# lucidrains/transfusion-pytorch

Measured on AMD Instinct MI355X. Metric: train samples/sec, dim512 d8 seq1024 text+latent, higher is better.
Workload: dtype bf16; 1 GPU; BASELINE config 2: Transfusion dim=512 depth=8 heads=8 dim_head=64 num_text_tokens=256 dim_latent=384; per-GPU batch 64 x seq 1024 (32 x [24 text tokens + (4,384) latent] per sample); step = pack + fwd + bwd + clip(0.5) + Adam(3e-4) (one GPU: no gradient exchange); global_batch=64, seq_len=1024, parallelism=dp1

## Files before the change

### include/tfx.h

```cpp
#ifndef TFX_H
#define TFX_H
#include <stdint.h>
#ifdef __cplusplus
extern "C" {
#endif

#ifndef TFX_BF16_DEFINED
typedef uint16_t tfx_bf16;
#endif

enum { TFX_EPI_BF16 = 0, TFX_EPI_F32 = 1, TFX_EPI_SILU = 2, TFX_EPI_RESID = 3, TFX_EPI_GEGLU = 4, TFX_EPI_GEGLU_BWD = 5, TFX_EPI_QKV_NORM_ROPE = 6 };

typedef struct {
  const tfx_bf16* A; int32_t lda;
  const tfx_bf16* A2; int32_t lda2; int32_t K1;
  const tfx_bf16* B; int32_t ldb;
  int32_t M, N, K;
  int32_t epi;
  void* C; int32_t ldc;
  void* C2; int32_t ldc2;
  const float* bias;
  const tfx_bf16* R; int32_t ldr; int32_t resid_mapped;
  const int32_t* rowmap;
  const int32_t* a_rowmap;
// ... 6 lines not shown
  tfx_bf16* qk_cache; int32_t qk_ld_cache; const int32_t* qk_cache_pos;
  const void* prefetch; int64_t prefetch_bytes;
} tfx_gemm_nt_args;
int tfx_gemm_nt(const tfx_gemm_nt_args* a, void* stream);
int tfx_gemm_nt_plan(const tfx_gemm_nt_args* a, int32_t* kind, int32_t* grid);

int tfx_mfma_peak_probe(const void* ops, float* out, int32_t iters, int32_t blocks, void* stream);

typedef struct {
  const tfx_bf16* A; int32_t lda; int32_t a_cols;
  const tfx_bf16* B; int32_t ldb; int32_t b_cols;
  int32_t M, N, K;
  float* C; int32_t ldc;
  const int32_t* rowmap;
  int32_t k_valid;
  int32_t splits;
  int32_t accumulate;
  float alpha;
  const int32_t* a_rowmap;
  const int32_t* b_rowmap;
  float* colsum;
  int32_t k_group;
  const void* group_next;
} tfx_gemm_tn_args;
int tfx_gemm_tn(const tfx_gemm_tn_args* a, void* stream);
int tfx_gemm_tn_plan(const tfx_gemm_tn_args* a, int32_t* kind, int32_t* tiles, int32_t* splits, int32_t* grid);

typedef struct {
  const tfx_bf16 *q, *k, *v; int32_t ld_q, ld_k, ld_v;
  const tfx_bf16* gate; int32_t ld_gate;
  const int32_t* kv_end;
  const int32_t* q_start;
  tfx_bf16* out; int32_t ld_out;
  float* lse;
  int32_t b, h, n;
  float softcap;
  int32_t n_kv;
  const tfx_bf16* dout; int32_t ld_dout;
  tfx_bf16* do_eff; int32_t ld_do;
  float* delta;
  tfx_bf16* dgate; int32_t ld_dgate;
  tfx_bf16 *dq, *dk, *dv; int32_t ld_dq, ld_dk, ld_dv;
  int32_t order;
  const float* sc_plan;
  const int32_t* q_row0; const int32_t* q_cnt;
  const tfx_bf16* nr_qkv; int32_t nr_ld_qkv;
// ... 296 lines not shown
```

### transfusion_pytorch_amd/csrc/gemm.hip

```cpp
#include "tfx_common.h"
#include "tfx_kernels.h"
#include <type_traits>
#include <cmath>
#include <cstring>
#include <vector>
#include <algorithm>
#include <mutex>

namespace tfx {

constexpr int BM = 128, BN = 128, BK = 64;

template <int EPI> struct Epilogue;

TFX_DEV void store_bf16x4(bf16* dst, f32x4 v) {
  bf16x4 o; o[0] = f2bf(v[0]); o[1] = f2bf(v[1]); o[2] = f2bf(v[2]); o[3] = f2bf(v[3]);
  *(bf16x4*)dst = o;
}

TFX_DEV f32x4 add_bias(const GemmNT& p, int n, f32x4 v) {
  if (p.bias) { f32x4 b = *(const f32x4*)(p.bias + n); v += b; }
  return v;
}

// ... 1884 lines not shown
#pragma unroll
      for (int j = 0; j < 4; j++)
        if (out_col[j] >= 0) atomicAdd(crow + out_col[j], acc[i][j][r] * p.alpha);
    }
  }
}
template <bool SUM>
__global__ __launch_bounds__(256, 1) void gemm_tn_ow_kernel(GemmTN p, int ramp) {
  const int ntn = (p.N + 255) / 256, ntk = (p.K + 255) / 256;
  tn_ow_body<SUM>(p, tn_block_ramp(p, ntn * ntk, ramp));
}
constexpr int TN_GROUP_MAX = 6;
struct TnGroup { int count; int tile_end[TN_GROUP_MAX]; GemmTN p[TN_GROUP_MAX]; };
template <bool SUM>
__global__ __launch_bounds__(256, 1) void gemm_tn_ow_group_kernel(TnGroup g, int ramp) {
  TnBlock blk = tn_block_ramp(g.p[0], g.tile_end[g.count - 1], ramp);
  int pid = 0, first = 0;
#pragma unroll
  for (int i = 0; i < TN_GROUP_MAX - 1; i++)
    if (i + 1 < g.count && blk.tile >= g.tile_end[i]) { pid = i + 1; first = g.tile_end[i]; }
  blk.tile -= first;
  tn_ow_body<SUM>(g.p[__builtin_amdgcn_readfirstlane(pid)], blk);
}
#undef OWT_OUT
#undef OWT_IN
#undef OWT_CLOBBER

static int tn_auto_splits(int M, int tiles, int kind) {
  constexpr double fill2 = 0.9, fill0 = 0.5;
  const int slots = kind == 2 ? 256 : 512;
  const double want = (kind == 2 ? fill2 : fill0) * slots;
  int s = 1;
  while (tiles * s < want && tiles * (s + 1) <= slots && s < 64 && M / (s + 1) >= 256) s++;
  return s;
}

static bool use_glds() {
  static int v = -1;
  if (v < 0) { const char* e = getenv("TFX_GEMM_GLDS"); v = (e && e[0] == '0') ? 0 : 1; }
  return v == 1;
}

enum { NT_FALLBACK = 0, NT_GLDS = 1, NT_MID = 2, NT_PP = 3, NT_SKINNY = 4, NT_DECODE = 5, NT_OW = 6, NT_OWP = 7 };

static const float* gelu_table() {
  static const float* tab[16] = {nullptr};
// ... 220 lines not shown
  const GemmTN* q = &head;
  int n = 0, tiles = 0;
  bool ok = grp != 0 && tn_ow_mode() != 0;
  while (q && n < TN_GROUP_MAX) {
    ok = ok && q->M == head.M && tn_ow_operands_ok(*q);
    tiles += ((q->N + 255) / 256) * ((q->K + 255) / 256);
    gp.g.p[n] = *q; gp.g.p[n].group_next = nullptr; gp.g.tile_end[n] = tiles;
    n++;
    q = (const GemmTN*)q->group_next;
  }
  ok = ok && q == nullptr && n >= 2;
  gp.count = n; gp.tiles = tiles; gp.g.count = n;
  if (!ok) return gp;
  gp.splits = head.splits == 0 ? tn_auto_splits(head.M, tiles, 2) : head.splits;
  const int chunk = ((head.M + gp.splits - 1) / gp.splits + TN_BMK - 1) / TN_BMK * TN_BMK;
  const int last = head.M % chunk == 0 ? chunk : head.M % chunk;
  if (chunk < 192 || last < 192) return gp;
  gp.grid = (tiles * gp.splits + 7) / 8 * 8;
  if (head.splits == 0 && tiles * gp.splits < 0.8 * 256) return gp;
  for (int i = 0; i < n; i++) gp.g.p[i].splits = gp.splits;
  gp.ok = true;
  return gp;
}
static int tn_ramp(int M, int tiles, int splits) {
  constexpr int ramp_min = 8;
  int ramp = 0;
  if (splits >= ramp_min && M % TN_BMK == 0) {
    const int S = splits, U = M / TN_BMK;
    ramp = (int)(0.148 * tiles + 0.5);
    while (ramp > 0 && (U - ramp * S * (S - 1) / 2) / S < 8) ramp--;
  }
  return ramp;
}

int gemm_tn_plan(const GemmTN& p, int* kind, int* tiles, int* splits, int* grid) {
  if (p.M <= 0 || p.N <= 0 || p.K <= 0 || p.splits < 0) return -1;
  if (p.group_next) {
    const TnGroupPlan gp = tn_group_plan(p);
    if (gp.ok) { if (kind) *kind = 3; if (tiles) *tiles = gp.tiles; if (splits) *splits = gp.splits; if (grid) *grid = gp.grid; return 0; }
  }
  const TnPlan pl = tn_plan(p);
  if (kind) *kind = pl.kind; if (tiles) *tiles = pl.tiles; if (splits) *splits = pl.splits; if (grid) *grid = pl.grid;
  return 0;
}

int gemm_tn(const GemmTN& p, hipStream_t s) {
  if (p.M <= 0 || p.N <= 0 || p.K <= 0 || p.splits < 0) return -1;
  if ((p.lda | p.ldb | p.a_cols | p.b_cols) & 7) return -2;
  if (p.group_next) {
    const TnGroupPlan gp = tn_group_plan(p);
    if (gp.ok) {
      bool sum = false;
      for (int i = 0; i < gp.count; i++) sum = sum || gp.g.p[i].colsum != nullptr;
      const int ramp = tn_ramp(p.M, gp.tiles, gp.splits);
      static uint32_t attr_g0 = 0, attr_g1 = 0;
      if (sum) { ensure_smem_attr((const void*)gemm_tn_ow_group_kernel<true>, 131072, attr_g1); hipLaunchKernelGGL(gemm_tn_ow_group_kernel<true>, dim3(gp.grid), dim3(256), 131072, s, gp.g, ramp); }
      else { ensure_smem_attr((const void*)gemm_tn_ow_group_kernel<false>, 131072, attr_g0); hipLaunchKernelGGL(gemm_tn_ow_group_kernel<false>, dim3(gp.grid), dim3(256), 131072, s, gp.g, ramp); }
      return (int)hipGetLastError();
    }
    int guard = 0;
    for (const GemmTN* q = &p; q; q = (const GemmTN*)q->group_next) {
      if (++guard > 64) return -7;
      GemmTN one = *q; one.group_next = nullptr;
      const int rc = gemm_tn(one, s);
      if (rc) return rc;
    }
    return 0;
  }
  static uint32_t attr_set = 0;
  const int smem = 2 * 2 * TN_BMK * TN_LD * 2;
  ensure_smem_attr((const void*)gemm_tn_kernel, smem, attr_set);
// ... 32 lines not shown
```

### transfusion_pytorch_amd/csrc/runner.hip

```cpp
#include <atomic>
#include <hip/hip_runtime.h>
#include <cstdlib>
#include <cstdint>
#include "../../include/tfx.h"

namespace {

inline int run_one(const tfx_launch& l, void* s) {
  const void* a = l.args;
  const tfx_raw_args* r = static_cast<const tfx_raw_args*>(a);
  switch (l.op) {
    case TFX_OP_GEMM_NT:          return tfx_gemm_nt(static_cast<const tfx_gemm_nt_args*>(a), s);
    case TFX_OP_GEMM_TN:          return tfx_gemm_tn(static_cast<const tfx_gemm_tn_args*>(a), s);
    case TFX_OP_ATTN_FWD:         return tfx_attn_fwd(static_cast<const tfx_attn_args*>(a), s);
    case TFX_OP_ATTN_BWD:         return tfx_attn_bwd(static_cast<const tfx_attn_args*>(a), s);
    case TFX_OP_ADALN_PRE_FWD:    return tfx_adaln_pre_fwd(static_cast<const tfx_adaln_pre_args*>(a), s);
    case TFX_OP_ADALN_PRE_BWD:    return tfx_adaln_pre_bwd(static_cast<const tfx_adaln_pre_args*>(a), s);
    case TFX_OP_ADALN_POST_FWD:   return tfx_adaln_post_fwd(static_cast<const tfx_adaln_post_args*>(a), s);
    case TFX_OP_ADALN_POST_BWD:   return tfx_adaln_post_bwd(static_cast<const tfx_adaln_post_args*>(a), s);
    case TFX_OP_QK_NORM_ROPE_FWD: return tfx_qk_norm_rope_fwd(static_cast<const tfx_qk_norm_rope_args*>(a), s);
    case TFX_OP_QK_NORM_ROPE_BWD: return tfx_qk_norm_rope_bwd(static_cast<const tfx_qk_norm_rope_args*>(a), s);
    case TFX_OP_ATTNRES_FWD:      return tfx_attnres_fwd(static_cast<const tfx_attnres_args*>(a), s);
    case TFX_OP_ATTNRES_BWD:      return tfx_attnres_bwd(static_cast<const tfx_attnres_args*>(a), s);
    case TFX_OP_RMSNORM_FWD:      return tfx_rmsnorm_fwd(static_cast<const tfx_rmsnorm_args*>(a), s);
// ... 192 lines not shown
extern "C" int tfx_list_fingerprint(const tfx_launch* list, int32_t n, int64_t* out) {
  if (!out || n < 0 || (n > 0 && !list)) return -1;
  uint64_t h = 1469598103934665603ull ^ (g_single_stream.load(std::memory_order_relaxed) ? 0x9e3779b97f4a7c15ull : 0ull);
  for (int32_t i = 0; i < n; ++i) {
    const tfx_launch& l = list[i];
    h = mix(h, &l.op, 4); h = mix(h, &l.stream, 4);
    if (l.op >= TFX_OP_FORK && l.op <= TFX_OP_JOIN_WAIT) continue;
    if (!l.args) return -2;
    const size_t nb = struct_bytes(l.op);
    if (nb == 0) return -100;
    h = mix(h, l.args, nb);
    const tfx_raw_args* r = static_cast<const tfx_raw_args*>(l.args);
    switch (l.op) {
      case TFX_OP_ADALN_POST_PRE_FWD: h = mix(h, r->p0, sizeof(tfx_adaln_post_args)); h = mix(h, r->p1, sizeof(tfx_adaln_pre_args)); break;
      case TFX_OP_LAYER_END_FWD:
        h = mix(h, r->p0, sizeof(tfx_adaln_post_args)); h = mix(h, r->p1, sizeof(tfx_attnres_args));
        if (r->p2) h = mix(h, r->p2, sizeof(tfx_adaln_pre_args));
        break;
      case TFX_OP_ATTNRES_PULL_BWD: h = mix(h, r->p0, sizeof(tfx_attnres_pull_args)); if (r->p1) h = mix(h, r->p1, sizeof(tfx_adaln_post_args)); break;
      case TFX_OP_ADALN_PRE_POST_BWD: h = mix(h, r->p0, sizeof(tfx_adaln_pre_args)); h = mix(h, r->p1, sizeof(tfx_adaln_post_args)); break;
      case TFX_OP_GEMM_TN: {
        const tfx_gemm_tn_args* g = static_cast<const tfx_gemm_tn_args*>(l.args);
        for (int k = 0; k < 8 && g->group_next; ++k) { g = static_cast<const tfx_gemm_tn_args*>(g->group_next); h = mix(h, g, sizeof(tfx_gemm_tn_args)); }
        break;
      }
      default: break;
    }
  }
  *out = (int64_t)h;
  return 0;
}

extern "C" int tfx_set_single_stream(int32_t on) {
  const int prev = g_single_stream.exchange(on != 0) ? 1 : 0;
  return prev;
}
```

### transfusion_pytorch_amd/csrc/tokenwise.hip

```cpp
#include "tfx_kernels.h"
#include <map>
#include <mutex>
#include <utility>
#include <cstdlib>

namespace tfx {

constexpr int WAVES = 4;
constexpr int MAXB = 1024;

template <int NC> struct Row {
  float v[NC][8];
};

template <int NC> TFX_DEV void load_row(Row<NC>& r, const bf16* p, int d, int lane) {
#pragma unroll
  for (int i = 0; i < NC; i++) {
    int c = lane + 64 * i;
    if (c * 8 < d) {
      bf16x8 x = *(const bf16x8*)(p + c * 8);
#pragma unroll
      for (int e = 0; e < 8; e++) r.v[i][e] = bf2f(x[e]);
    } else {
#pragma unroll
// ... 2324 lines not shown
int tfx_attn_fwd(const tfx_attn_args* a, void* s) { return attn_fwd(*a, ST(s)); }
int tfx_attn_bwd(const tfx_attn_args* a, void* s) { return attn_bwd(*a, ST(s)); }
int tfx_mfma_peak_probe(const void* ops, float* out, int32_t iters, int32_t blocks, void* s) {
  if (!ops || !out || iters <= 0 || blocks <= 0) return -1;
  hipLaunchKernelGGL(mfma_peak_k, dim3(blocks), dim3(256), 0, ST(s), (const bf16x8*)ops, out, iters); RET();
}
int tfx_laser_v_fwd(const tfx_laser_v_args* a, void* s) {
  if (!a || a->T < 0 || a->H <= 0 || !(a->c > 0.f)) return -1;
  if (a->T == 0) return 0;
  if (!a->v || !a->vl || ((a->ld_v | a->ld_vl) & 7) || a->ld_v < a->H * 64 || a->ld_vl < a->H * 64 || (((uintptr_t)a->v | (uintptr_t)a->vl) & 15)) return -2;
  const long long nch = (long long)a->T * a->H * 8;
  if (nch >= (1ll << 31)) return -4;
  hipLaunchKernelGGL(laser_v_fwd_k, dim3((unsigned)((nch + 255) / 256)), dim3(256), 0, ST(s), *a, (unsigned)nch); RET();
}
int tfx_laser_v_bwd(const tfx_laser_v_args* a, void* s) {
  if (!a || a->T < 0 || a->H <= 0 || !(a->c > 0.f)) return -1;
  if (a->T == 0) return 0;
  if (!a->v || !a->dvl || !a->dv || ((a->ld_v | a->ld_dvl | a->ld_dv) & 7) || a->ld_v < a->H * 64 || a->ld_dvl < a->H * 64 || a->ld_dv < a->H * 64 ||
      (((uintptr_t)a->v | (uintptr_t)a->dvl | (uintptr_t)a->dv) & 15)) return -2;
  const long long nch = (long long)a->T * a->H * 8;
  if (nch >= (1ll << 31)) return -4;
  hipLaunchKernelGGL(laser_v_bwd_k, dim3((unsigned)((nch + 255) / 256)), dim3(256), 0, ST(s), *a, (unsigned)nch); RET();
}
const char* tfx_version(void) { return "tfx-hip gfx950 r5-laser-muon-selfflow-adamgroups-oderk"; }

}
```

### transfusion_pytorch_amd/engine.py

```python
from __future__ import annotations

import ctypes
import os
import weakref

import torch

from . import capi
from .params import ModelDims, ParamStore, pad_to

BF16 = torch.bfloat16
E = capi.ENUMS


def _p(t, *idx):
    for i in idx:
        t = t[i]
    return t.data_ptr()


def skip_sources(md: ModelDims):
    stack, src = [], {}
    for i in range(md.depth):
        layer = i + 1
# ... 114 lines not shown
                    arr[k].stream = int(a)
                    arr[k].args = ctypes.addressof(_DUMMY)
                    continue
                arr[k].stream = 1 if isinstance(item, Side) else 0
                if isinstance(fn, str):
                    arr[k].op = capi.ENUMS['TFX_OP_' + fn[4:].upper()]
                    arr[k].args = ctypes.addressof(a)
                else:
                    name = fn.__name__
                    r = raw_args(name, a)
                    keep.append(r)
                    if isinstance(a, list):
                        live.append((name, a, r))
                    arr[k].op = capi.ENUMS['TFX_OP_' + name[4:].upper()]
                    arr[k].args = ctypes.addressof(r)
            self._image = (len(self), arr, keep, live)
        for name, a, r in self._image[3]:
            fresh = raw_args(name, a)
            ctypes.memmove(ctypes.addressof(r), ctypes.addressof(fresh), ctypes.sizeof(_RAW))
        return self._image[1]


class Plan:
    def __init__(self, ps: ParamStore, b: int, n: int, I: int, R: dict, training: bool = True, cache=None, dp_groups: int = 0, tile_attn: bool = False, units=None, ctl_rows: int = 2):
        md = ps.md
        self.units = units
        assert not units or (cache is not None and tile_attn), 'compacted plans are decode plans on the tiled attention kernel (the row ranges are its arguments)'
        self.cache = cache
        self.tile_attn = tile_attn
        assert cache is None or not training
        self.dp_groups = dp_groups
        self.bwd_cuts = []
        self.ps, self.md, self.b, self.n, self.I, self.R = ps, md, b, n, I, dict(R)
        self.T = T = b * n
        dev = ps.device
        d, hd, D, dip, ldq, nt3 = md.dim, md.hdk, md.depth, md.dip, md.ldq, md.nt3
        self.nbytes = 0
        def z(*s, dtype=BF16):
            t = torch.zeros(*s, device=dev, dtype=dtype); self.nbytes += t.numel() * t.element_size(); return t
        def e(*s, dtype=BF16):
            t = torch.empty(*s, device=dev, dtype=dtype); self.nbytes += t.numel() * t.element_size(); return t
        I1 = max(I, 1)
        self.idx = z(7, max(T, 1, 4 * units[0] if units else 1), dtype=torch.int32)
        self.text_ids, self.cache_pos, self.kv_end, self.rot_pos, self.tok_inst, self.q_start, self.labels = (self.idx[r, :T] if r != 1 else self.idx[r] for r in range(7))
        if units:
            U = units[0]
            self.unit_row0, self.unit_cnt, self.unit_blk0, self.unit_txt = (self.idx[6, k * U:(k + 1) * U] for k in range(4))
        self.inst_time = z(I1, dtype=torch.float32)
        self.row_tok = {t: z(r, dtype=torch.int32) for t, r in R.items()}
        self.rowbuf = None
        if cache is not None and R and len(set(R.values())) == 1:
            r = next(iter(R.values()))
            self.row_stride = rs = (r + 3) // 4 * 4
            self.rowbuf = z(2 * len(R) * rs + ctl_rows * max(b, units[0] if units else 0), dtype=torch.int32)
            self.row_tok = {t: self.rowbuf[k * rs:k * rs + r] for k, t in enumerate(R)}
# ... 42 lines not shown
                self.vl = e(nl, T, hd)
            else:
                side = ps.__dict__.setdefault('_laser_side', weakref.WeakValueDictionary())
                key = (cache.data_ptr(), tuple(cache.shape), tuple(cache.stride()))
                self.vlc = side.get(key)
                if self.vlc is None:
                    self.vlc = e(D, cache.shape[1] * cache.shape[2], hd)
                    side[key] = self.vlc
        self.fwd, self.bwd = LaunchList(), LaunchList()
        self.noise_args = {}
        self.loaded_structure = None
        self._seg_args = []
        self.seg_start = z(max(T, 1), dtype=torch.int32); self.seg_len = z(max(T, 1), dtype=torch.int32)
        self.pull = training and D <= 32 and md.dim <= 1024
        if self.pull:
            self.arsave = [e(T, i + 2, 4, dtype=torch.float32) for i in range(D)]
            self.arerr = e(D, T, d)
        self._build_forward()
        if training:
            self.dH = e(D + 1, T, d)
            self.gx = {i: e(T, d) for i in range(D) if md.has_skip(i)}; self.du = e(T, d)
            env = os.environ.get('TFX_SIDE_STREAM')
            self.side = D <= 30 and (env == '1' or (env is None and md.dim <= 1024))
            nb = 2 if self.side else 1
            self.dy_f = [e(T, d) for _ in range(nb)]; self.dy_a = [e(T, d) for _ in range(nb)] if self.side else self.dy_f
            self.dskip = {j: e(T, d) for j in set(skip_sources(md).values())}
            self.dqkvg_p = [z(T, ldq) for _ in range(nb)]; self.dog = e(T, hd); self.do_eff = e(T, hd)
            self.dqk = e(T, 2 * hd) if os.environ.get('TFX_ATTN_QKNR', '1') == '0' else None
            self.delta = e(b, md.heads, n, dtype=torch.float32)
            self.dag_p = [e(T, 2 * dip) for _ in range(nb)]; self.dembed = e(T, d); self.gfin = e(T, d); self.dx0 = e(T, d)
            self.dtables = z(I1, nt3, dtype=torch.float32); self.dtab_bf = e(I1, nt3)
            self.dcond = e(I1, 4 * d); self.dpre = e(I1, 4 * d)
            self.onehot = e(T, md.vp)
            self._build_backward()

    def _nt(self, lst, algo_n=None, algo_k=None, **kw):
        a = capi.make_args('tfx_gemm_nt_args', **kw)
        a._algo_flops = 2.0 * kw['M'] * (algo_n or kw['N']) * (algo_k or kw['K'])
        lst.append(('tfx_gemm_nt', a))

    def _tn(self, lst, M, N, K, **kw):
        splits = 0
        kw.setdefault('k_valid', K)
        algo_n = kw.pop('algo_n', None)
        side = kw.pop('side', False)
        a = capi.make_args('tfx_gemm_tn_args', M=M, N=N, K=K, splits=splits, accumulate=1, alpha=1.0, **kw)
        a._algo_flops = 2.0 * M * (algo_n or N) * kw['k_valid']
        lst.append(Side(('tfx_gemm_tn', a)) if side else ('tfx_gemm_tn', a))

    def _tn_group(self, lst, M, problems, side=False):
        if len(problems) < 2 or os.environ.get('TFX_TN_GROUP', '1') == '0':
            for (N, K, kw) in problems:
                self._tn(lst, M, N, K, side=side, **kw)
            return
        structs, flops = [], 0.0
        for (N, K, kw) in problems:
            kw = dict(kw); kw.setdefault('k_valid', K)
            algo_n = kw.pop('algo_n', None)
            a = capi.make_args('tfx_gemm_tn_args', M=M, N=N, K=K, splits=0, accumulate=1, alpha=1.0, **kw)
            flops += 2.0 * M * (algo_n or N) * kw['k_valid']
            structs.append(a)
        for a, b in zip(structs, structs[1:]):
            a.group_next = ctypes.addressof(b)
        head = structs[0]
        head._chain = structs[1:]
        head._algo_flops = flops
        lst.append(Side(('tfx_gemm_tn', head)) if side else ('tfx_gemm_tn', head))

    def _k(self, lst, fn, struct, **kw):
        lst.append((fn, capi.make_args(struct, **kw)))

    def _raw(self, lst, fn, *args):
        lst.append((fn, args))

    def _hbm(self, lst, passes, extra_bytes=0):
        if lst.meta is None:
            lst.meta = {}
        lst.meta[len(lst) - 1] = ('hbm', passes * self.T * self.md.dim * 2 + extra_bytes)

    def _tab(self, i, w):
        off = ((i * 2 + w) * 3 * self.md.dim) * 4
        return self.tables.data_ptr() + off, (self.dtables.data_ptr() + off if hasattr(self, 'dtables') else 0)

    def _build_forward(self):
        ps, md, T, I = self.ps, self.md, self.T, self.I
        d, hd, D, dip, ldq, nt3, H = md.dim, md.hdk, md.depth, md.dip, md.ldq, md.nt3, md.heads
        S = ps.shadows
        L = self.fwd
        pp = ps.ptr
        if self.cache is not None:
# ... 220 lines not shown
        assert mode in ('latent', 'model')
        self.clean_mode = mode
        for t, a in self._clean_launch.items():
            lt = self.lat[t]
            a[1] = lt['q'].data_ptr() if mode == 'model' else lt['x'].data_ptr()
            a[2] = None if mode == 'model' else self.noise_args[t].eps

    def _attn_kw(self, i, bwd=False):
        md, hd, ldq = self.md, self.md.hdk, self.md.ldq
        li, lkv = self._li(i), self._lkv(i)
        kw = dict(q=self.qkr[lkv], k=_p(self.qkr, lkv) + 2 * hd, v=_p(self.qkvg, lkv) + 2 * 2 * hd, ld_q=2 * hd, ld_k=2 * hd, ld_v=ldq,
                  gate=_p(self.qkvg, lkv) + 2 * 3 * hd, ld_gate=ldq, kv_end=self.kv_end, q_start=self.q_start, out=self.og[li], ld_out=hd,
                  lse=self.lse[li], b=self.units[0] if self.units else self.b, h=md.heads, n=self.units[1] if self.units else self.n, softcap=50.0)
        if self.units:
            kw.update(q_row0=self.unit_row0, q_cnt=self.unit_cnt)
        if self.sc_plan is not None:
            kw['sc_plan'] = self.sc_plan[i]
        if self.cache is not None:
            ck = self.cache[i]
            kw.update(k=ck.data_ptr(), v=ck.data_ptr() + 2 * hd, ld_k=2 * hd, ld_v=2 * hd, n_kv=int(ck.shape[1]))
        if md.laser:
            kw.update(v=self.vl[li] if self.cache is None else self.vlc[i], ld_v=hd, laser=1)
        if bwd:
            dqkvg = self.dqkvg_p[i % len(self.dqkvg_p)]
            kw.update(dout=self.dog, ld_dout=hd, do_eff=self.do_eff, ld_do=hd, delta=self.delta,
                      dgate=dqkvg.data_ptr() + 2 * 3 * hd, ld_dgate=ldq, dq=self.dqk if self.dqk is not None else 0,
                      dk=self.dqk.data_ptr() + 2 * hd if self.dqk is not None else 0,
                      dv=dqkvg.data_ptr() + 2 * 2 * hd, ld_dq=2 * hd, ld_dk=2 * hd, ld_dv=ldq)
        return kw

    def set_rope_tables(self, cos_tab, sin_tab):
        if self.cos_tab is not None and (self.cos_tab.data_ptr() != cos_tab.data_ptr() or self.sin_tab.data_ptr() != sin_tab.data_ptr()):
            self.fwd.invalidate_graphs()
        self.cos_tab, self.sin_tab = cos_tab, sin_tab
        for a in getattr(self, '_rope_args', []):
            a.cos_tab, a.sin_tab = cos_tab.data_ptr(), sin_tab.data_ptr()
        for a in getattr(self, '_rope_nt_args', []):
            a.qk_cos, a.qk_sin = cos_tab.data_ptr(), sin_tab.data_ptr()
        for a in getattr(self, '_rope_attn_args', []):
            a.nr_cos, a.nr_sin = cos_tab.data_ptr(), sin_tab.data_ptr()

    def set_segments(self, seg_start, seg_len):
        n_seg = int(seg_start.numel())
        self.seg_start[:n_seg].copy_(seg_start); self.seg_len[:n_seg].copy_(seg_len)
        for a in self._seg_args:
            a.n_seg = n_seg

# ... 107 lines not shown
                                 pq=pp(f'{pj}.pseudo_queries'), dgamma=gp(f'{pj}.norm_keys.gamma'), dpq=gp(f'{pj}.pseudo_queries'), L=j + 2).items():
                    setattr(recs[j], k, v.data_ptr() if hasattr(v, 'data_ptr') else v)
            raw = torch.frombuffer(bytearray(ctypes.string_at(ctypes.addressof(recs), ctypes.sizeof(recs))), dtype=torch.uint8)
            self._src_tab = raw.to(ps.device)
            self._src_size = ctypes.sizeof(SRC)
            self._raw(L, lib.tfx_attnres_prep, self._src_tab.data_ptr(), D, d)
        self._pull_args = {}
        def pull_launch(l, out_own, add, dh, post):
            j0 = max(l - 1, 0)
            ns = D - j0
            export = ns > 8 or d > 512
            if export and not hasattr(self, 'k1buf'):
                self.k1buf = torch.zeros(T, 32, device=ps.device, dtype=BF16); self.nbytes += self.k1buf.numel() * 2
            a = capi.make_args('tfx_attnres_pull_args', T=T, d=d, l=l, n_src=ns, h=self.hid[l], src=self._src_tab.data_ptr() + j0 * self._src_size,
                               out_own=out_own, out_err=self.arerr[l - 1] if out_own is not None else None, add=add, dh=dh,
                               seg_start=self.seg_start, seg_len=self.seg_len, n_seg=0, k1=self.k1buf if export else None, ld_k1=32)
            self._seg_args.append(a)
            self._pull_args[l] = a
            self._keep = getattr(self, '_keep', []) + [a, post]
            self._raw(L, lib.tfx_attnres_pull_bwd, ctypes.addressof(a), ctypes.addressof(post) if post is not None else None)
            self._hbm(L, ns + 6 if post is not None else ns + 4, 12 * ns * T)
            if export:
                self._tn(L, T, ns, d, A=self.k1buf, lda=32, a_cols=32, B=self.hid[l], ldb=d, b_cols=d, C=self.wtab[1, j0], ldc=d)
        for i in range(D - 1, -1, -1):
            p = f'transformer.layers.{i}'
            x_in = self.xres[i]
            x_a = self.xa[i] if md.has_skip(i) else x_in
            (ta, dta), (tf, dtf) = self._tab(i, 0), self._tab(i, 1)
            par = i % len(self.dag_p)
            dy_f, dy_a, dag, dqkvg = self.dy_f[par], self.dy_a[par], self.dag_p[par], self.dqkvg_p[par]
            if i + 2 <= D - 1:
                sync('tfx_join_wait', i + 2)
            G = self.dH[i + 1]
            a_postf = capi.make_args('tfx_adaln_post_args', T=T, d=d, y=self.yf[i], tok_inst=self.tok_inst, table=tf, ld_table=nt3,
                                     layerscale=pp(f'{p}.2.layerscale'), g=G, dy=dy_f, dtable=dtf, dlayerscale=gp(f'{p}.2.layerscale'),
                                     seg_start=self.seg_start, seg_len=self.seg_len, n_seg=0, dbias=gp(f'{p}.2.fn.net.3.bias'))
            self._seg_args.append(a_postf)
            if pull:
                pull_launch(i + 1, self.xres[i + 1], None, G, a_postf)
            else:
                g2 = self.dskip[i + 1] if (i + 1) in pushed else None
                self._k(L, 'tfx_attnres_bwd', 'tfx_attnres_args', T=T, d=d, L=i + 2, hiddens=self.hid, stride_h=T * d,
                        gamma=pp(f'{p}.3.norm_keys.gamma'), pq=pp(f'{p}.3.pseudo_queries'), g=g, g2=capi.ptr(g2), dhiddens=self.dH, stride_dh=T * d,
                        first=1 if i == D - 1 else 0, dgamma=gp(f'{p}.3.norm_keys.gamma'), dpq=gp(f'{p}.3.pseudo_queries'))
                L.append(('tfx_adaln_post_bwd', a_postf))
            self._nt(L, algo_n=di, A=dy_f, lda=d, B=S[f'ff2_t{i}'], ldb=d, M=T, N=dip, K=d, epi=E['TFX_EPI_GEGLU_BWD'], C=dag, ldc=2 * dip,
                     aux=self.ag[i], ldaux=2 * dip)
            sync('tfx_fork', 2 * i)
            ff_grp = [(d, di, dict(A=dy_f, lda=d, a_cols=d, B=self.hm[i], ldb=dip, b_cols=dip, C=gp(f'{p}.2.fn.net.3.weight'), ldc=di)),
                      (2 * dip, d, dict(algo_n=2 * di, A=dag, lda=2 * dip, a_cols=2 * dip, B=self.uf[i], ldb=d, b_cols=d, rowmap=gmap,
                                        C=gp(f'{p}.2.fn.net.0.weight'), ldc=d, colsum=gp(f'{p}.2.fn.net.0.bias')))]
            self._tn_group(L, T, ff_grp, side=side)
            self._nt(L, algo_k=2 * di, A=dag, lda=2 * dip, B=S[f'ff1_t{i}'], ldb=2 * dip, M=T, N=d, K=2 * dip, epi=E['TFX_EPI_BF16'], C=self.du, ldc=d)
            a_pref = capi.make_args('tfx_adaln_pre_args', T=T, d=d, x=self.xb[i], tok_inst=self.tok_inst, table=tf, ld_table=nt3,
                                    gamma_text=pp(f'{p}.2.layernorm_gamma'), mean=_p(self.stats, 2, i), rstd=_p(self.stats, 3, i), du=self.du, dx=G,
                                    dtable=dtf, dgamma_text=gp(f'{p}.2.layernorm_gamma'), seg_start=self.seg_start, seg_len=self.seg_len, n_seg=0)
            a_posta = capi.make_args('tfx_adaln_post_args', T=T, d=d, y=self.ya[i], tok_inst=self.tok_inst, table=ta, ld_table=nt3,
                                     layerscale=pp(f'{p}.1.layerscale'), g=G, dy=dy_a, dtable=dta, dlayerscale=gp(f'{p}.1.layerscale'),
                                     seg_start=self.seg_start, seg_len=self.seg_len, n_seg=0)
            self._seg_args += [a_pref, a_posta]
            self._keep = getattr(self, '_keep', []) + [a_pref, a_posta]
            self._raw(L, lib.tfx_adaln_pre_post_bwd, ctypes.addressof(a_pref), ctypes.addressof(a_posta))
            self._hbm(L, 6)
            self._nt(L, algo_n=md.hd, A=dy_a, lda=d, B=S[f'out_t{i}'], ldb=d, M=T, N=hd, K=d, epi=E['TFX_EPI_BF16'], C=self.dog, ldc=hd)
            gam = (lambda nm: S[f'g{nm}{i}']) if md.dim_head != 64 else (lambda nm: pp(f'{p}.1.fn.{nm}_norm.gamma'))
            if os.environ.get('TFX_ATTN_QKNR', '1') != '0':
                self._k(L, 'tfx_attn_bwd', 'tfx_attn_args', **self._attn_kw(i, bwd=True), nr_qkv=self.qkvg[i], nr_ld_qkv=ldq, nr_dqkv=dqkvg, nr_ld_dqkv=ldq,
                        nr_gamma_q=gam('q'), nr_gamma_k=gam('k'), nr_rot_pos=self.rot_pos, nr_cos=0, nr_sin=0, nr_q_scale=md.dim_head ** -0.5,
                        nr_norm_scale=md.dim_head ** 0.5, nr_dgamma_q=gp(f'{p}.1.fn.q_norm.gamma'), nr_dgamma_k=gp(f'{p}.1.fn.k_norm.gamma'))
                self._rope_attn_args = getattr(self, '_rope_attn_args', []) + [L[-1][1]]
            else:
                self._k(L, 'tfx_attn_bwd', 'tfx_attn_args', **self._attn_kw(i, bwd=True))
                self._k(L, 'tfx_qk_norm_rope_bwd', 'tfx_qk_norm_rope_args', T=T, H=H, qkv=self.qkvg[i], ld_qkv=ldq, gamma_q=gam('q'),
                        gamma_k=gam('k'), rot_pos=self.rot_pos, cos_tab=0, sin_tab=0, q_scale=md.dim_head ** -0.5, norm_scale=md.dim_head ** 0.5,
                        dqk=self.dqk, ld_dqk=2 * hd, dqkv=dqkvg, ld_dqkv=ldq, dgamma_q=gp(f'{p}.1.fn.q_norm.gamma'), dgamma_k=gp(f'{p}.1.fn.k_norm.gamma'))
                self._rope_args = getattr(self, '_rope_args', []) + [L[-1][1]]
                L.meta = L.meta or {}
                L.meta[len(L) - 1] = ('hbm', 3 * 2 * T * hd * 2)
            if md.laser:
                dv = dqkvg.data_ptr() + 2 * 2 * hd
                self._k(L, 'tfx_laser_v_bwd', 'tfx_laser_v_args', T=T, H=H, v=_p(self.qkvg, i) + 2 * 2 * hd, ld_v=ldq, c=md.laser,
                        dvl=dv, ld_dvl=ldq, dv=dv, ld_dv=ldq)
                L.meta = L.meta or {}
                L.meta[len(L) - 1] = ('hbm', 3 * T * hd * 2)
            self._nt(L, algo_k=md.nq, A=dqkvg, lda=ldq, B=S[f'qkvg_t{i}'], ldb=ldq, M=T, N=d, K=ldq, epi=E['TFX_EPI_BF16'], C=self.du, ldc=d)
            self._k(L, 'tfx_adaln_pre_bwd', 'tfx_adaln_pre_args', T=T, d=d, x=x_a, tok_inst=self.tok_inst, table=ta, ld_table=nt3,
                    gamma_text=pp(f'{p}.1.layernorm_gamma'), mean=_p(self.stats, 0, i), rstd=_p(self.stats, 1, i), du=self.du, dx=G,
                    dtable=dta, dgamma_text=gp(f'{p}.1.layernorm_gamma'), seg_start=self.seg_start, seg_len=self.seg_len, n_seg=0,
                    dx_add=self.dskip[i] if (pull and i in pushed) else None)
            self._hbm(L, 4 + (1 if (pull and i in pushed) else 0))
            self._seg_args.append(L[-1][1])
            sync('tfx_fork', 2 * i + 1)
            grp = [(d, hd, dict(A=dy_a, lda=d, a_cols=d, B=self.og[i], ldb=hd, b_cols=hd, C=gp(f'{p}.1.fn.to_out.1.weight'), ldc=md.hd,
                                k_group=0 if md.dim_head == 64 else md.dim_head)),
                   (md.nqk, d, dict(algo_n=md.nq, A=dqkvg, lda=ldq, a_cols=ldq, B=self.ua[i], ldb=d, b_cols=d, C=gp(f'{p}.1.fn.to_qk.0.weight'), ldc=d,
                                    rowmap=ps._maps['heads'] if md.dim_head != 64 else None))]
            if md.has_skip(i):
                sk = self.xres[src[i]]
                grp.append((d, d, dict(A=G, lda=d, a_cols=d, B=x_in, ldb=d, b_cols=d, C=gp(f'{p}.0.weight'), ldc=2 * d)))
                grp.append((d, d, dict(A=G, lda=d, a_cols=d, B=sk, ldb=d, b_cols=d, C=gp(f'{p}.0.weight', d), ldc=2 * d)))
            self._tn_group(L, T, grp, side=side)
            per = -(-D // self.dp_groups) if self.dp_groups > 0 else D
            if I > 0 and i % per == 0:
                hi = min(i + per, D)
                off, cols = i * 2 * 3 * d, (hi - i) * 2 * 3 * d
                w_item = lambda it: L.append(Side(it) if side else it)
                w_item((lib.tfx_cast_block_bf16, (self.dtables.data_ptr() + 4 * off, nt3, self.dtab_bf.data_ptr() + 2 * off, nt3, I, cols)))
                self._tn(L, I, cols, 4 * d, side=side, A=self.dtab_bf.data_ptr() + 2 * off, lda=nt3, a_cols=cols, B=self.cond, ldb=4 * d, b_cols=4 * d,
                         C=gp(f'{p}.1.to_film.weight'), ldc=4 * d)
                w_item((lib.tfx_colsum_f32, (self.dtables.data_ptr() + 4 * off, nt3, I, cols, gp(f'{p}.1.to_film.bias'))))
            sync('tfx_join_record', i)
            if self.dp_groups > 0:
                if i % per == 0:
                    sync('tfx_join_wait', i)
                    self.bwd_cuts.append((len(L), i, min(i + per, D) - 1))
            if md.has_skip(i):
                st = S[f'skip_t{i}']
                self._nt(L, A=G, lda=d, B=st, ldb=d, M=T, N=d, K=d, epi=E['TFX_EPI_RESID'], C=self.gx[i], ldc=d, R=G, ldr=d)
                self._nt(L, A=G, lda=d, B=st[d:], ldb=d, M=T, N=d, K=d, epi=E['TFX_EPI_BF16'], C=self.dskip[src[i]], ldc=d)
                g = self.gx[i]
            else:
                g = G
        sync('tfx_join', 63)
        if pull:
            pull_launch(0, None, g, self.dx0, None)
            self._raw(L, lib.tfx_attnres_finish, self._src_tab.data_ptr(), D, d)
        else:
            self._raw(L, lib.tfx_add_bf16, g.data_ptr(), self.dH[0].data_ptr(), self.dx0.data_ptr(), T * d)
            if 0 in pushed:
                self._raw(L, lib.tfx_add_bf16, self.dx0.data_ptr(), self.dskip[0].data_ptr(), self.dx0.data_ptr(), T * d)
        self._raw(L, lib.tfx_onehot_bf16, self.text_ids.data_ptr(), self.tok_inst.data_ptr(), self.onehot.data_ptr(), T, md.vp)
        self._x0_param_grads(L, self.dx0)
        if I > 0:
            self._nt(L, A=self.dtab_bf, lda=nt3, B=S['ada_t'], ldb=nt3, M=I, N=4 * d, K=nt3, epi=E['TFX_EPI_BF16'], C=self.dcond, ldc=4 * d)
# ... 114 lines not shown
```

Measured before the change: 2542 samples/s.

## Batch weight-gradient GEMMs across layers into one device-table TN launch

Adds a table-driven TN GEMM kernel that reads per-problem argument records from device memory, so weight-gradient GEMMs from many layers can run in a single launch. The planner defers the per-layer FF and attention weight-gradient groups and launches them as one table at the end of a run of layers, with one side-stream fork and join per run instead of per layer. It also adds a split-count cost model for the table kernel. To keep deferred operands alive, more gradient buffers are allocated (up to depth rather than 2), which adds memory use and delays the overlap of weight-gradient work with the main stream.

```diff
diff --git a/include/tfx.h b/include/tfx.h
--- a/include/tfx.h
+++ b/include/tfx.h
@@ -52,6 +52,10 @@
   float* colsum;
   int32_t k_group;
   const void* group_next;
+  const void* table;
+  const void* table_host;
+  int32_t table_count;
+  int32_t table_reserved;
 } tfx_gemm_tn_args;
 int tfx_gemm_tn(const tfx_gemm_tn_args* a, void* stream);
 int tfx_gemm_tn_plan(const tfx_gemm_tn_args* a, int32_t* kind, int32_t* tiles, int32_t* splits, int32_t* grid);
diff --git a/transfusion_pytorch_amd/csrc/gemm.hip b/transfusion_pytorch_amd/csrc/gemm.hip
--- a/transfusion_pytorch_amd/csrc/gemm.hip
+++ b/transfusion_pytorch_amd/csrc/gemm.hip
@@ -1930,6 +1930,35 @@
   blk.tile -= first;
   tn_ow_body<SUM>(g.p[__builtin_amdgcn_readfirstlane(pid)], blk);
 }
+constexpr int TN_REC_WORDS = (int)(sizeof(GemmTN) / 4);
+static_assert(sizeof(GemmTN) % 8 == 0, "records are copied as 32-bit words and followed by an int32 array");
+template <bool SUM>
+__global__ __launch_bounds__(256, 1) void gemm_tn_ow_table_kernel(const uint32_t* __restrict__ recs, const int* __restrict__ tile_end, int count, int M, int splits) {
+  const int per = gridDim.x >> 3;
+  const int g = (int)(blockIdx.x & 7) * per + (int)(blockIdx.x >> 3);
+  int lo = 0, hi = count;
+  while (lo < hi) {
+    const int mid = (lo + hi) >> 1;
+    if (g >= splits * tile_end[mid]) lo = mid + 1; else hi = mid;
+  }
+  if (lo >= count) return;
+  const int r = __builtin_amdgcn_readfirstlane(lo);
+  const int first = r > 0 ? tile_end[r - 1] : 0, nt = tile_end[r] - first;
+  const int local = g - splits * first;
+  const int split = local / nt;
+  const int chunk = ((M + splits - 1) / splits + TN_BMK - 1) / TN_BMK * TN_BMK;
+  TnBlock blk;
+  blk.tile = local - split * nt;
+  blk.mbeg = min(split * chunk, M);
+  blk.mend = min(M, blk.mbeg + chunk);
+  uint32_t w[TN_REC_WORDS];
+#pragma unroll
+  for (int i = 0; i < TN_REC_WORDS; i++) w[i] = __builtin_amdgcn_readfirstlane(recs[(size_t)r * TN_REC_WORDS + i]);
+  GemmTN p;
+  __builtin_memcpy(&p, w, sizeof(GemmTN));
+  if (p.M != M) return;
+  tn_ow_body<SUM>(p, blk);
+}
 #undef OWT_OUT
 #undef OWT_IN
 #undef OWT_CLOBBER
@@ -2196,6 +2225,47 @@
   gp.ok = true;
   return gp;
 }
+static int tn_table_splits(int M, int tiles) {
+  constexpr double atom_rows = 9.5;
+  int best = 1; double best_cost = -1;
+  for (int s = 1; s <= 256; s++) {
+    const int chunk = ((M + s - 1) / s + TN_BMK - 1) / TN_BMK * TN_BMK;
+    if (s > 1 && chunk < 256) break;
+    if ((long long)(s - 1) * chunk >= M) continue;
+    if (M - (s - 1) * chunk < 192) continue;
+    const double cost = (double)(((long long)tiles * s + 255) / 256) * chunk + atom_rows * tiles * s;
+    if (best_cost < 0 || cost < best_cost) { best = s; best_cost = cost; }
+  }
+  return best;
+}
+struct TnTablePlan { bool ok, sum; int tiles, splits, grid; };
+static const GemmTN* tn_table_rec(const GemmTN& head, int i) { return (const GemmTN*)head.table_host + i; }
+static TnTablePlan tn_table_plan(const GemmTN& head) {
+  TnTablePlan tp; memset(&tp, 0, sizeof(tp));
+  static int tab = -1;
+  if (tab < 0) { const char* e = getenv("TFX_TN_TABLE"); tab = e ? atoi(e) : 1; }
+  const int n = head.table_count;
+  const int32_t* tile_end = (const int32_t*)(tn_table_rec(head, n));
+  bool ok = tab != 0 && tn_ow_mode() != 0 && (((uintptr_t)head.table) & 7) == 0;
+  int tiles = 0;
+  for (int i = 0; i < n; i++) {
+    const GemmTN* q = tn_table_rec(head, i);
+    ok = ok && q->M == head.M && tn_ow_operands_ok(*q);
+    tiles += ((q->N + 255) / 256) * ((q->K + 255) / 256);
+    ok = ok && tile_end[i] == tiles;
+    tp.sum = tp.sum || q->colsum != nullptr;
+  }
+  tp.tiles = tiles;
+  if (!ok) return tp;
+  tp.splits = head.splits == 0 ? tn_table_splits(head.M, tiles) : head.splits;
+  const int chunk = ((head.M + tp.splits - 1) / tp.splits + TN_BMK - 1) / TN_BMK * TN_BMK;
+  const int last = head.M % chunk == 0 ? chunk : head.M % chunk;
+  if (chunk < 192 || last < 192) return tp;
+  if ((long long)tiles * tp.splits > (1ll << 30)) return tp;
+  tp.grid = (tiles * tp.splits + 7) / 8 * 8;
+  tp.ok = true;
+  return tp;
+}
 static int tn_ramp(int M, int tiles, int splits) {
   constexpr int ramp_min = 8;
   int ramp = 0;
@@ -2209,7 +2279,11 @@
 
 int gemm_tn_plan(const GemmTN& p, int* kind, int* tiles, int* splits, int* grid) {
   if (p.M <= 0 || p.N <= 0 || p.K <= 0 || p.splits < 0) return -1;
-  if (p.group_next) {
+  if (p.table) {
+    if (!p.table_host || p.table_count <= 0) return -8;
+    const TnTablePlan tp = tn_table_plan(p);
+    if (tp.ok) { if (kind) *kind = 3; if (tiles) *tiles = tp.tiles; if (splits) *splits = tp.splits; if (grid) *grid = tp.grid; return 0; }
+  } else if (p.group_next) {
     const TnGroupPlan gp = tn_group_plan(p);
     if (gp.ok) { if (kind) *kind = 3; if (tiles) *tiles = gp.tiles; if (splits) *splits = gp.splits; if (grid) *grid = gp.grid; return 0; }
   }
@@ -2221,6 +2295,24 @@
 int gemm_tn(const GemmTN& p, hipStream_t s) {
   if (p.M <= 0 || p.N <= 0 || p.K <= 0 || p.splits < 0) return -1;
   if ((p.lda | p.ldb | p.a_cols | p.b_cols) & 7) return -2;
+  if (p.table) {
+    if (!p.table_host || p.table_count <= 0) return -8;
+    const TnTablePlan tp = tn_table_plan(p);
+    if (tp.ok) {
+      const uint32_t* recs = (const uint32_t*)p.table;
+      const int* tile_end = (const int*)((const GemmTN*)p.table + p.table_count);
+      static uint32_t attr_t0 = 0, attr_t1 = 0;
+      if (tp.sum) { ensure_smem_attr((const void*)gemm_tn_ow_table_kernel<true>, 131072, attr_t1); hipLaunchKernelGGL(gemm_tn_ow_table_kernel<true>, dim3(tp.grid), dim3(256), 131072, s, recs, tile_end, p.table_count, p.M, tp.splits); }
+      else { ensure_smem_attr((const void*)gemm_tn_ow_table_kernel<false>, 131072, attr_t0); hipLaunchKernelGGL(gemm_tn_ow_table_kernel<false>, dim3(tp.grid), dim3(256), 131072, s, recs, tile_end, p.table_count, p.M, tp.splits); }
+      return (int)hipGetLastError();
+    }
+    for (int i = 0; i < p.table_count; i++) {
+      GemmTN one = *tn_table_rec(p, i); one.group_next = nullptr; one.table = nullptr; one.table_host = nullptr; one.table_count = 0;
+      const int rc = gemm_tn(one, s);
+      if (rc) return rc;
+    }
+    return 0;
+  }
   if (p.group_next) {
     const TnGroupPlan gp = tn_group_plan(p);
     if (gp.ok) {
diff --git a/transfusion_pytorch_amd/csrc/runner.hip b/transfusion_pytorch_amd/csrc/runner.hip
--- a/transfusion_pytorch_amd/csrc/runner.hip
+++ b/transfusion_pytorch_amd/csrc/runner.hip
@@ -238,6 +238,8 @@
       case TFX_OP_GEMM_TN: {
         const tfx_gemm_tn_args* g = static_cast<const tfx_gemm_tn_args*>(l.args);
         for (int k = 0; k < 8 && g->group_next; ++k) { g = static_cast<const tfx_gemm_tn_args*>(g->group_next); h = mix(h, g, sizeof(tfx_gemm_tn_args)); }
+        const tfx_gemm_tn_args* t = static_cast<const tfx_gemm_tn_args*>(l.args);
+        if (t->table && t->table_host && t->table_count > 0) h = mix(h, t->table_host, (size_t)t->table_count * (sizeof(tfx_gemm_tn_args) + 4));
         break;
       }
       default: break;
diff --git a/transfusion_pytorch_amd/csrc/tokenwise.hip b/transfusion_pytorch_amd/csrc/tokenwise.hip
--- a/transfusion_pytorch_amd/csrc/tokenwise.hip
+++ b/transfusion_pytorch_amd/csrc/tokenwise.hip
@@ -2370,6 +2370,6 @@
   if (nch >= (1ll << 31)) return -4;
   hipLaunchKernelGGL(laser_v_bwd_k, dim3((unsigned)((nch + 255) / 256)), dim3(256), 0, ST(s), *a, (unsigned)nch); RET();
 }
-const char* tfx_version(void) { return "tfx-hip gfx950 r5-laser-muon-selfflow-adamgroups-oderk"; }
-
-}
+const char* tfx_version(void) { return "tfx-hip gfx950 r5-laser-muon-selfflow-adamgroups-oderk-tntable"; }
+
+}
diff --git a/transfusion_pytorch_amd/engine.py b/transfusion_pytorch_amd/engine.py
--- a/transfusion_pytorch_amd/engine.py
+++ b/transfusion_pytorch_amd/engine.py
@@ -160,7 +160,7 @@
 
 
 class Plan:
-    def __init__(self, ps: ParamStore, b: int, n: int, I: int, R: dict, training: bool = True, cache=None, dp_groups: int = 0, tile_attn: bool = False, units=None, ctl_rows: int = 2):
+    def __init__(self, ps: ParamStore, b: int, n: int, I: int, R: dict, training: bool = True, cache=None, dp_groups: int = 0, tile_attn: bool = False, units=None, ctl_rows: int = 2, tn_defer=None):
         md = ps.md
         self.units = units
         assert not units or (cache is not None and tile_attn), 'compacted plans are decode plans on the tiled attention kernel (the row ranges are its arguments)'
@@ -169,6 +169,7 @@
         assert cache is None or not training
         self.dp_groups = dp_groups
         self.bwd_cuts = []
+        self.tn_defer = tn_defer
         self.ps, self.md, self.b, self.n, self.I, self.R = ps, md, b, n, I, dict(R)
         self.T = T = b * n
         dev = ps.device
@@ -257,8 +258,10 @@
             self.gx = {i: e(T, d) for i in range(D) if md.has_skip(i)}; self.du = e(T, d)
             env = os.environ.get('TFX_SIDE_STREAM')
             self.side = D <= 30 and (env == '1' or (env is None and md.dim <= 1024))
-            nb = 2 if self.side else 1
-            self.dy_f = [e(T, d) for _ in range(nb)]; self.dy_a = [e(T, d) for _ in range(nb)] if self.side else self.dy_f
+            self.tn_run = self._tn_run_length()
+            self.tn_tables = []
+            nb = min(D, 2 * self.tn_run) if self.tn_run else (2 if self.side else 1)
+            self.dy_f = [e(T, d) for _ in range(nb)]; self.dy_a = [e(T, d) for _ in range(nb)] if (self.side or self.tn_run) else self.dy_f
             self.dskip = {j: e(T, d) for j in set(skip_sources(md).values())}
             self.dqkvg_p = [z(T, ldq) for _ in range(nb)]; self.dog = e(T, hd); self.do_eff = e(T, hd)
             self.dqk = e(T, 2 * hd) if os.environ.get('TFX_ATTN_QKNR', '1') == '0' else None
@@ -301,6 +304,53 @@
         head._chain = structs[1:]
         head._algo_flops = flops
         lst.append(Side(('tfx_gemm_tn', head)) if side else ('tfx_gemm_tn', head))
+
+    def _tn_run_length(self):
+        md, D = self.md, self.md.depth
+        v = self.tn_defer if self.tn_defer is not None else os.environ.get('TFX_TN_DEFER')
+        if v is not None and str(v) != '':
+            return D if str(v) == 'all' else max(0, min(int(v), D))
+        if os.environ.get('TFX_TN_GROUP', '1') == '0' or md.dim > 512:
+            return 0
+        d, hd, di, dip, ldq = md.dim, md.hdk, md.di, md.dip, md.ldq
+        mk = lambda N, K, lda, ldb: capi.make_args('tfx_gemm_tn_args', M=self.T, N=N, K=K, lda=lda, a_cols=lda, ldb=ldb, b_cols=ldb, ldc=K, k_valid=K, splits=0,
+                                                   accumulate=1, alpha=1.0)
+        for chain in ([mk(d, di, d, dip), mk(2 * dip, d, 2 * dip, d)], [mk(d, hd, d, hd), mk(md.nqk, d, ldq, d)]):
+            chain[0].group_next = ctypes.addressof(chain[1])
+            out = [ctypes.c_int32(-9) for _ in range(4)]
+            if capi.lib().tfx_gemm_tn_plan(ctypes.byref(chain[0]), *[ctypes.byref(o) for o in out]) != 0:
+                return 0
+            tiles = sum(-(-int(a.N) // 256) * -(-int(a.K) // 256) for a in chain)
+            if out[0].value != 3 or out[1].value != tiles:
+                return 0
+        return D
+
+    def _bwd_slot(self, i):
+        nb = len(self.dag_p)
+        return (self.md.depth - 1 - i) % nb if self.tn_run else i % nb
+
+    def _tn_table(self, lst, M, problems, side=False):
+        REC = capi.STRUCTS['tfx_gemm_tn_args']
+        n, rs = len(problems), ctypes.sizeof(REC)
+        host = ctypes.create_string_buffer(n * (rs + 4))
+        ends = (ctypes.c_int32 * n).from_buffer(host, n * rs)
+        flops, tiles = 0.0, 0
+        for k, (N, K, kw) in enumerate(problems):
+            kw = dict(kw); kw.setdefault('k_valid', K)
+            algo_n = kw.pop('algo_n', None)
+            a = capi.make_args('tfx_gemm_tn_args', M=M, N=N, K=K, splits=0, accumulate=1, alpha=1.0, **kw)
+            flops += 2.0 * M * (algo_n or N) * kw['k_valid']
+            ctypes.memmove(ctypes.addressof(host) + k * rs, ctypes.addressof(a), rs)
+            tiles += -(-N // 256) * -(-K // 256)
+            ends[k] = tiles
+        dev = torch.frombuffer(bytearray(host.raw), dtype=torch.uint8).to(self.ps.device)
+        self.nbytes += dev.numel()
+        head = REC.from_buffer_copy(host, 0)
+        head.table, head.table_host, head.table_count = dev.data_ptr(), ctypes.addressof(host), n
+        head._table = (host, dev)
+        head._algo_flops = flops
+        lst.append(Side(('tfx_gemm_tn', head)) if side else ('tfx_gemm_tn', head))
+        return dev
 
     def _k(self, lst, fn, struct, **kw):
         lst.append((fn, capi.make_args(struct, **kw)))
@@ -567,7 +617,7 @@
         if md.laser:
             kw.update(v=self.vl[li] if self.cache is None else self.vlc[i], ld_v=hd, laser=1)
         if bwd:
-            dqkvg = self.dqkvg_p[i % len(self.dqkvg_p)]
+            dqkvg = self.dqkvg_p[self._bwd_slot(i)]
             kw.update(dout=self.dog, ld_dout=hd, do_eff=self.do_eff, ld_do=hd, delta=self.delta,
                       dgate=dqkvg.data_ptr() + 2 * 3 * hd, ld_dgate=ldq, dq=self.dqk if self.dqk is not None else 0,
                       dk=self.dqk.data_ptr() + 2 * hd if self.dqk is not None else 0,
@@ -721,15 +771,24 @@
             self._hbm(L, ns + 6 if post is not None else ns + 4, 12 * ns * T)
             if export:
                 self._tn(L, T, ns, d, A=self.k1buf, lda=32, a_cols=32, B=self.hid[l], ldb=d, b_cols=d, C=self.wtab[1, j0], ldc=d)
+        run, pending = self.tn_run, []
+        run_low = {}
+        if run:
+            per_g = -(-D // self.dp_groups) if self.dp_groups > 0 else D
+            for j in range(D - 1, -1, -1):
+                top = min((j // per_g + 1) * per_g, D) - 1
+                run_low[j] = max(top - ((top - j) // run + 1) * run + 1, j // per_g * per_g)
         for i in range(D - 1, -1, -1):
             p = f'transformer.layers.{i}'
             x_in = self.xres[i]
             x_a = self.xa[i] if md.has_skip(i) else x_in
             (ta, dta), (tf, dtf) = self._tab(i, 0), self._tab(i, 1)
-            par = i % len(self.dag_p)
+            par = self._bwd_slot(i)
             dy_f, dy_a, dag, dqkvg = self.dy_f[par], self.dy_a[par], self.dag_p[par], self.dqkvg_p[par]
-            if i + 2 <= D - 1:
+            if not run and i + 2 <= D - 1:
                 sync('tfx_join_wait', i + 2)
+            if run and i + len(self.dag_p) <= D - 1:
+                sync('tfx_join_wait', run_low[i + len(self.dag_p)])
             G = self.dH[i + 1]
             a_postf = capi.make_args('tfx_adaln_post_args', T=T, d=d, y=self.yf[i], tok_inst=self.tok_inst, table=tf, ld_table=nt3,
                                      layerscale=pp(f'{p}.2.layerscale'), g=G, dy=dy_f, dtable=dtf, dlayerscale=gp(f'{p}.2.layerscale'),
@@ -745,11 +804,15 @@
                 L.append(('tfx_adaln_post_bwd', a_postf))
             self._nt(L, algo_n=di, A=dy_f, lda=d, B=S[f'ff2_t{i}'], ldb=d, M=T, N=dip, K=d, epi=E['TFX_EPI_GEGLU_BWD'], C=dag, ldc=2 * dip,
                      aux=self.ag[i], ldaux=2 * dip)
-            sync('tfx_fork', 2 * i)
+            if not run:
+                sync('tfx_fork', 2 * i)
             ff_grp = [(d, di, dict(A=dy_f, lda=d, a_cols=d, B=self.hm[i], ldb=dip, b_cols=dip, C=gp(f'{p}.2.fn.net.3.weight'), ldc=di)),
                       (2 * dip, d, dict(algo_n=2 * di, A=dag, lda=2 * dip, a_cols=2 * dip, B=self.uf[i], ldb=d, b_cols=d, rowmap=gmap,
                                         C=gp(f'{p}.2.fn.net.0.weight'), ldc=d, colsum=gp(f'{p}.2.fn.net.0.bias')))]
-            self._tn_group(L, T, ff_grp, side=side)
+            if run:
+                pending += ff_grp
+            else:
+                self._tn_group(L, T, ff_grp, side=side)
             self._nt(L, algo_k=2 * di, A=dag, lda=2 * dip, B=S[f'ff1_t{i}'], ldb=2 * dip, M=T, N=d, K=2 * dip, epi=E['TFX_EPI_BF16'], C=self.du, ldc=d)
             a_pref = capi.make_args('tfx_adaln_pre_args', T=T, d=d, x=self.xb[i], tok_inst=self.tok_inst, table=tf, ld_table=nt3,
                                     gamma_text=pp(f'{p}.2.layernorm_gamma'), mean=_p(self.stats, 2, i), rstd=_p(self.stats, 3, i), du=self.du, dx=G,
@@ -789,7 +852,10 @@
                     dx_add=self.dskip[i] if (pull and i in pushed) else None)
             self._hbm(L, 4 + (1 if (pull and i in pushed) else 0))
             self._seg_args.append(L[-1][1])
-            sync('tfx_fork', 2 * i + 1)
+            per = -(-D // self.dp_groups) if self.dp_groups > 0 else D
+            launch = bool(run) and run_low[i] == i
+            if not run or launch:
+                sync('tfx_fork', 2 * i + 1)
             grp = [(d, hd, dict(A=dy_a, lda=d, a_cols=d, B=self.og[i], ldb=hd, b_cols=hd, C=gp(f'{p}.1.fn.to_out.1.weight'), ldc=md.hd,
                                 k_group=0 if md.dim_head == 64 else md.dim_head)),
                    (md.nqk, d, dict(algo_n=md.nq, A=dqkvg, lda=ldq, a_cols=ldq, B=self.ua[i], ldb=d, b_cols=d, C=gp(f'{p}.1.fn.to_qk.0.weight'), ldc=d,
@@ -798,8 +864,14 @@
                 sk = self.xres[src[i]]
                 grp.append((d, d, dict(A=G, lda=d, a_cols=d, B=x_in, ldb=d, b_cols=d, C=gp(f'{p}.0.weight'), ldc=2 * d)))
                 grp.append((d, d, dict(A=G, lda=d, a_cols=d, B=sk, ldb=d, b_cols=d, C=gp(f'{p}.0.weight', d), ldc=2 * d)))
-            self._tn_group(L, T, grp, side=side)
-            per = -(-D // self.dp_groups) if self.dp_groups > 0 else D
+            if run:
+                pending += grp
+                if launch:
+                    hi_l = max(j for j in run_low if run_low[j] == i)
+                    self.tn_tables.append((len(L), i, hi_l, self._tn_table(L, T, pending, side=side), len(pending)))
+                    pending = []
+            else:
+                self._tn_group(L, T, grp, side=side)
             if I > 0 and i % per == 0:
                 hi = min(i + per, D)
                 off, cols = i * 2 * 3 * d, (hi - i) * 2 * 3 * d
@@ -808,7 +880,8 @@
                 self._tn(L, I, cols, 4 * d, side=side, A=self.dtab_bf.data_ptr() + 2 * off, lda=nt3, a_cols=cols, B=self.cond, ldb=4 * d, b_cols=4 * d,
                          C=gp(f'{p}.1.to_film.weight'), ldc=4 * d)
                 w_item((lib.tfx_colsum_f32, (self.dtables.data_ptr() + 4 * off, nt3, I, cols, gp(f'{p}.1.to_film.bias'))))
-            sync('tfx_join_record', i)
+            if not run or launch:
+                sync('tfx_join_record', i)
             if self.dp_groups > 0:
                 if i % per == 0:
                     sync('tfx_join_wait', i)
```

New measurement: 2580 samples/s (median of 6 runs). 1.01x the previous value.
